# czbiohub-sf/shrimPy

Measured on AMD Instinct MI355X. Metric: voxels/sec deskew+20-iter RL deconv, 2048×2048×512 f32; HBM GB/s vs peak, higher is better.
Workload: dtype f32

## Files before the change

shrimpy_amd/csrc/rfft_rows.hip:

```cpp

#include "correlate_common.hpp"
#include "fft_lds.hpp"

namespace {

using namespace lsr_fft;

constexpr int kThreads = 512;
constexpr int kRows = 8;
constexpr int kPerRow = kThreads / kRows;
constexpr int kMaxM = 2048;
constexpr int kMaxTapsX = 2 * kPerRow + 1;

struct RowsArgs {
  const float* in;
  int Zi, Yi, Xi;
  float2* spec;
  int Z, Y, X, M, XC;
  const float2* tw_half;
  const float2* tw_x;
  Factors f;
  float* pval;
  unsigned long long* pidx;
  const float* aux;
  float* out;
  int Zo, Yo, Xo;
  float scale, eps;
  int pz, py, px;
  const double* norm_table;
  float norm_full;
  double* stats;
};

__device__ __forceinline__ int reflect_index(int i, int n) {
  if (n == 1) return 0;
  const int period = 2 * (n - 1);
  i = i % period;
  if (i < 0) i += period;
  return i < n ? i : period - i;
}
__device__ __forceinline__ int match_index(int o, int ni, int no) {
  if (no > ni) return reflect_index(o - (no - ni) / 2, ni);
  return o + (ni - no) / 2;
}

struct Tile {
  float2* buf;
  float2* tw;
  int pitch;
};

__device__ __forceinline__ Tile carve(float2* smem, int M) {
  Tile t;
  t.pitch = M + 1;
  t.buf = smem;
  t.tw = smem + kRows * t.pitch;
  return t;
}

__device__ __forceinline__ float2 tw_m(const float2* tw, int half, int i) {
  const bool hi = i >= half;
  const float2 v = tw[hi ? i - half : i];
  return hi ? float2{-v.x, -v.y} : v;
}

__device__ __forceinline__ int xcd_tile(int n_tiles, int block) {
  const int per = (n_tiles + 7) >> 3;
  const int t = (block & 7) * per + (block >> 3);
  return t < n_tiles ? t : -1;
}
__host__ __device__ inline unsigned xcd_grid(int64_t n_tiles) { return static_cast<unsigned>(8 * ((n_tiles + 7) / 8)); }

__device__ __forceinline__ void store_zero_tile(const RowsArgs& p, int z, int y0, int nrows, int tid) {
  const int r = tid & (kRows - 1), k0 = tid / kRows;
  if (r < nrows) {
    float2* out = p.spec + static_cast<int64_t>(z) * p.XC * p.Y + y0 + r;
    for (int k = k0; k <= p.M; k += kThreads / kRows) out[static_cast<int64_t>(k) * p.Y] = float2{0.0f, 0.0f};
  }
}

__device__ __forceinline__ void r2c_post_store(const RowsArgs& p, const Tile& t, int z, int y0, int nrows, int tid) {
  const int M = p.M;
  const int r = tid & (kRows - 1), k0 = tid / kRows;
  if (r < nrows) {
    const float2* row = t.buf + r * t.pitch;
    float2* out = p.spec + static_cast<int64_t>(z) * p.XC * p.Y + y0 + r;
    const float2* twx = p.tw_x;
    const int64_t ystride = p.Y;
    batched_loop<8>(k0, M + 1, kThreads / kRows, [twx](int k) { return twx[k]; },
                    [row, out, M, ystride](int k, float2 w) {
                      const float2 a = row[k == M ? 0 : k], b = cconj(row[k == 0 ? 0 : M - k]);
                      const float2 e = float2{0.5f * (a.x + b.x), 0.5f * (a.y + b.y)};
                      const float2 o = mul_mi(float2{0.5f * (a.x - b.x), 0.5f * (a.y - b.y)});
                      out[static_cast<int64_t>(k) * ystride] = cadd(e, cmul(w, o));
                    });
  }
}

template <bool ZERO>
__global__ __launch_bounds__(kThreads) void rfft_rows_kernel(RowsArgs p) {
  extern __shared__ float2 smem[];
  const int M = p.M, half = M / 2;
  const Tile t = carve(smem, M);
  const int tid = threadIdx.x;
  const int tiles_y = (p.Y + kRows - 1) / kRows;
  int z, y0;
  if constexpr (ZERO) {
    const int ty_src = (p.Yi + kRows - 1) / kRows, n_src = p.Zi * ty_src;
    const int first_pad = static_cast<int>(xcd_grid(n_src));
    if (static_cast<int>(blockIdx.x) < first_pad) {
      const int tile = xcd_tile(n_src, blockIdx.x);
      if (tile < 0) return;
      z = tile / ty_src;
      y0 = (tile - z * ty_src) * kRows;
    } else {
      const int q = static_cast<int>(blockIdx.x) - first_pad, beside = tiles_y - ty_src, n_beside = p.Zi * beside;
      if (q >= n_beside) return;
      z = q / beside;
      y0 = (ty_src + q - z * beside) * kRows;
    }
  } else {
    const int tile = xcd_tile(p.Z * tiles_y, blockIdx.x);
    if (tile < 0) return;
    z = tile / tiles_y;
    y0 = (tile - z * tiles_y) * kRows;
  }
  const int nrows = min(kRows, p.Y - y0);

  if constexpr (ZERO) {
    if (z >= p.Zi || y0 >= p.Yi) {
      store_zero_tile(p, z, y0, nrows, tid);
      return;
    }
  }
  for (int k = tid; k < half; k += kThreads) t.tw[k] = p.tw_half[k];
  if constexpr (ZERO) {
    const int r = tid / kPerRow, lane = tid & (kPerRow - 1);
    float2* row = t.buf + r * t.pitch;
    if (r < nrows && y0 + r < p.Yi) {
      const float* src = p.in + (static_cast<int64_t>(z) * p.Yi + y0 + r) * p.Xi;
      const int last = p.Xi - 1, n_src = (p.Xi + 1) / 2;
      batched_loop<8>(lane, n_src, kPerRow,
                      [src, last](int m) { return float2{src[2 * m], src[min(2 * m + 1, last)]}; },
                      [row, last](int m, float2 v) { row[m] = float2{v.x, 2 * m + 1 <= last ? v.y : 0.0f}; });
      for (int m = lane + ((n_src - lane + kPerRow - 1) / kPerRow) * kPerRow; m < M; m += kPerRow) row[m] = float2{0.0f, 0.0f};
    } else {
      for (int m = lane; m < M; m += kPerRow) row[m] = float2{0.0f, 0.0f};
    }
  } else {
    const int r = tid / kPerRow, lane = tid & (kPerRow - 1);
    float2* row = t.buf + r * t.pitch;
    if (r < nrows) {
      const float* src = p.in + (static_cast<int64_t>(match_index(z, p.Zi, p.Z)) * p.Yi + match_index(y0 + r, p.Yi, p.Y)) * p.Xi;
      const int shift = p.X > p.Xi ? -((p.X - p.Xi) / 2) : (p.Xi - p.X) / 2;
      const int xi = p.Xi;
      batched_loop<8>(lane, M, kPerRow,
                      [src, shift, xi](int m) {
                        const int x0 = 2 * m + shift, x1 = x0 + 1;
                        const bool inside = x0 >= 0 && x1 < xi;
                        return float2{src[inside ? x0 : reflect_index(x0, xi)], src[inside ? x1 : reflect_index(x1, xi)]};
                      },
                      [row](int m, float2 v) { row[m] = v; });
    } else {
      for (int m = lane; m < M; m += kPerRow) row[m] = float2{0.0f, 0.0f};
    }
  }
  __syncthreads();

  const float2* twl = t.tw;
  transform<kMaxM, kPerRow>(t.buf + (tid / kPerRow) * t.pitch, M, p.f, [twl, half](int i) { return tw_m(twl, half, i); },
                            tid & (kPerRow - 1));

  __syncthreads();
  r2c_post_store(p, t, z, y0, nrows, tid);
}

__device__ __forceinline__ void load_spectrum_tile(const RowsArgs& p, const Tile& t, int z, int y0, int y_end, int tid) {
  const int M = p.M;
  const int r = tid & (kRows - 1), k0 = tid / kRows;
  float2* row = t.buf + r * t.pitch;
  if (y0 + r < y_end) {
    const float2* in = p.spec + static_cast<int64_t>(z) * p.XC * p.Y + y0 + r;
    const int64_t ystride = p.Y;
    batched_loop<10>(k0, M + 1, kThreads / kRows, [in, ystride](int k) { return in[static_cast<int64_t>(k) * ystride]; },
                     [row](int k, float2 v) { row[k] = v; });
  } else {
    for (int k = k0; k <= M; k += kThreads / kRows) row[k] = float2{0.0f, 0.0f};
  }
}

__device__ __forceinline__ void c2r_pre_step(const RowsArgs& p, const Tile& t, int tid) {
  const int M = p.M, half = M / 2;
  const int r = tid / kPerRow, lane = tid & (kPerRow - 1);
  float2* row = t.buf + r * t.pitch;
  const float2* twx = p.tw_x;
  struct Pair { float2 a, b; };
  batched_loop<5>(lane, half + 1, kPerRow, [twx, M](int m) { return Pair{twx[m], twx[M - m]}; },
                  [row, M](int m, Pair w) {
                    const int mm = M - m;
                    const float2 xa = row[m], xb = row[mm];
                    const float2 wa = cconj(w.a), wb = cconj(w.b);
                    const float2 za = cadd(cadd(xa, cconj(xb)), mul_i(cmul(wa, csub(xa, cconj(xb)))));
                    const float2 zb = cadd(cadd(xb, cconj(xa)), mul_i(cmul(wb, csub(xb, cconj(xa)))));
                    row[m] = cconj(za);
                    if (m != 0 && mm != m) row[mm] = cconj(zb);
                  });
}

__device__ __forceinline__ void peak_merge(float& v, unsigned long long& i, float v2, unsigned long long i2) {
  if (v2 > v || (v2 == v && i2 < i)) { v = v2; i = i2; }
}

__global__ __launch_bounds__(kThreads) void irfft_rows_peak_kernel(RowsArgs p) {
  extern __shared__ float2 smem[];
  const int M = p.M, half = M / 2;
  const Tile t = carve(smem, M);
  unsigned long long* const s_i = reinterpret_cast<unsigned long long*>(smem);
  float* const s_v = reinterpret_cast<float*>(smem + kThreads);
  const int tid = threadIdx.x;
  const int tiles_y = (p.Y + kRows - 1) / kRows;
  const int z = blockIdx.x / tiles_y, y0 = (blockIdx.x - z * tiles_y) * kRows;
  const int nrows = min(kRows, p.Y - y0);

  for (int k = tid; k < half; k += kThreads) t.tw[k] = p.tw_half[k];
  load_spectrum_tile(p, t, z, y0, p.Y, tid);
  __syncthreads();
  c2r_pre_step(p, t, tid);
  __syncthreads();

  const float2* twl = t.tw;
  transform<kMaxM, kPerRow>(t.buf + (tid / kPerRow) * t.pitch, M, p.f, [twl, half](int i) { return tw_m(twl, half, i); },
                            tid & (kPerRow - 1));

  float best = -1.0f;
  unsigned long long best_i = ~0ull;
  {
    const int r = tid / kPerRow, lane = tid & (kPerRow - 1);
    if (r < nrows) {
      const float2* row = t.buf + r * t.pitch;
      const int y = y0 + r;
      const int zs = (z + p.Z / 2) % p.Z, ys = (y + p.Y / 2) % p.Y;
      const unsigned long long base = (static_cast<unsigned long long>(zs) * p.Y + ys) * p.X;
      for (int m = lane; m < M; m += kPerRow) {
        const float2 v = row[m];
        const float a = fabsf(v.x), b = fabsf(v.y);
        if (a >= best) peak_merge(best, best_i, a, base + static_cast<unsigned>((2 * m + p.X / 2) % p.X));
        if (b >= best) peak_merge(best, best_i, b, base + static_cast<unsigned>((2 * m + 1 + p.X / 2) % p.X));
      }
    }
  }
  __syncthreads();
  s_v[tid] = best;
  s_i[tid] = best_i;
  __syncthreads();
  for (int w = kThreads / 2; w > 0; w >>= 1) {
    if (tid < w) peak_merge(s_v[tid], s_i[tid], s_v[tid + w], s_i[tid + w]);
    __syncthreads();
  }
  if (tid == 0) {
    p.pval[blockIdx.x] = s_v[0];
    p.pidx[blockIdx.x] = s_i[0];
  }
}

__device__ __forceinline__ float rl_border_norm(const RowsArgs& p, int z, int y, int x) {
  const double* P = p.norm_table;
  const int cz = p.pz / 2, cy = p.py / 2, cx = p.px / 2;
  const int a0 = max(0, cz - z), a1 = min(p.pz, p.Zo - z + cz);
  const int b0 = max(0, cy - y), b1 = min(p.py, p.Yo - y + cy);
  const int c0 = max(0, cx - x), c1 = min(p.px, p.Xo - x + cx);
  const int sb = p.px + 1, sa = (p.py + 1) * sb;
  return static_cast<float>(((P[a1 * sa + b1 * sb + c1] - P[a0 * sa + b1 * sb + c1]) -
                             (P[a1 * sa + b0 * sb + c1] - P[a0 * sa + b0 * sb + c1])) -
                            ((P[a1 * sa + b1 * sb + c0] - P[a0 * sa + b1 * sb + c0]) -
                             (P[a1 * sa + b0 * sb + c0] - P[a0 * sa + b0 * sb + c0])));
}

template <int EPI, bool STATS, bool CHAIN = false>
__global__ __launch_bounds__(kThreads) void irfft_rows_rl_kernel(RowsArgs p) {
  extern __shared__ float2 smem[];
  const int M = p.M, half = M / 2;
  const Tile t = carve(smem, M);
  const int tid = threadIdx.x;
  const int ty_out = (p.Yo + kRows - 1) / kRows, n_out = p.Zo * ty_out;
  int z, y0;
  if (!CHAIN || static_cast<int>(blockIdx.x) < static_cast<int>(xcd_grid(n_out))) {
    const int tile = xcd_tile(n_out, blockIdx.x);
    if (tile < 0) return;
    z = tile / ty_out;
    y0 = (tile - z * ty_out) * kRows;
  } else {
    const int tiles_y = (p.Y + kRows - 1) / kRows;
    const int q = static_cast<int>(blockIdx.x) - static_cast<int>(xcd_grid(n_out)), beside = tiles_y - ty_out;
    const int n_beside = p.Zo * beside;
    if (q < n_beside) {
      z = q / beside;
      y0 = (ty_out + q - z * beside) * kRows;
      store_zero_tile(p, z, y0, min(kRows, p.Y - y0), tid);
    }
    return;
  }
  const int nrows = min(kRows, p.Yo - y0);

  for (int k = tid; k < half; k += kThreads) t.tw[k] = p.tw_half[k];
  load_spectrum_tile(p, t, z, y0, p.Y, tid);
  __syncthreads();
  c2r_pre_step(p, t, tid);
  __syncthreads();

  float n_left[2] = {1.0f, 1.0f}, n_right[2] = {1.0f, 1.0f}, n_row = 1.0f;
  int m_right = -1;
  if constexpr (EPI == LSR_EPI_UPDATE) {
    const int r = tid / kPerRow, lane = tid & (kPerRow - 1);
    if (r < nrows) {
      const int y = y0 + r;
      const int cz = p.pz / 2, cy = p.py / 2, cx = p.px / 2;
      const bool zy_inside = z >= cz && z < p.Zo - cz && y >= cy && y < p.Yo - cy;
      n_row = zy_inside ? p.norm_full : rl_border_norm(p, z, y, min(cx, p.Xo - 1));
      const int m_lo = max(p.Xo - cx, 0) >> 1, m_hi = (p.Xo - 1) >> 1;
      m_right = m_lo + ((lane - m_lo) & (kPerRow - 1));
      if (m_right > m_hi) m_right = -1;
#pragma unroll
      for (int h = 0; h < 2; ++h) {
        const int xl = 2 * lane + h, xr = 2 * m_right + h;
        n_left[h] = (xl < cx && xl < p.Xo) ? rl_border_norm(p, z, y, xl) : n_row;
        n_right[h] = (m_right >= 0 && xr >= p.Xo - cx && xr < p.Xo) ? rl_border_norm(p, z, y, xr) : n_row;
      }
    }
  }

  const float2* twl = t.tw;
  transform<kMaxM, kPerRow>(t.buf + (tid / kPerRow) * t.pitch, M, p.f, [twl, half](int i) { return tw_m(twl, half, i); },
                            tid & (kPerRow - 1));

  lsr::RlStats stats;
  {
    const int r = tid / kPerRow, lane = tid & (kPerRow - 1);
    if (r < nrows) {
      float2* row = t.buf + r * t.pitch;
      const int y = y0 + r;
      const int64_t base = (static_cast<int64_t>(z) * p.Yo + y) * p.Xo;
      const float* aux = p.aux + base;
      float* out = p.out == nullptr ? nullptr : p.out + base;
      const int cx = p.px / 2;
      const int last = p.Xo - 1;
      batched_loop<6>(lane, (p.Xo + 1) / 2, kPerRow,
                      [aux, last](int m) { return float2{aux[2 * m], aux[min(2 * m + 1, last)]}; },
                      [&](int m, float2 av) {
        const float2 c = row[m];
        const float v[2] = {c.x * p.scale, -c.y * p.scale};
        const float a2[2] = {av.x, av.y};
        float res[2] = {0.0f, 0.0f};
#pragma unroll
        for (int h = 0; h < 2; ++h) {
          const int x = 2 * m + h;
          if (x < p.Xo) {
            const float a = a2[h];
            if constexpr (EPI == LSR_EPI_RATIO) {
              res[h] = a / (fmaxf(v[h], 0.0f) + p.eps);
              if (!CHAIN || out != nullptr) out[x] = res[h];
            } else {
              const float nrm = (m == lane && x < cx) ? n_left[h] : ((m == m_right && x >= p.Xo - cx) ? n_right[h] : n_row);
              const float xu = a * v[h];
              res[h] = xu / nrm;
              out[x] = res[h];
              if constexpr (STATS) stats.add(a, xu, res[h]);
            }
          }
        }
        if constexpr (CHAIN) row[m] = float2{res[0], res[1]};
      });
      if constexpr (CHAIN) {
        const int n_src = (p.Xo + 1) / 2;
        for (int m = lane + ((n_src - lane + kPerRow - 1) / kPerRow) * kPerRow; m < M; m += kPerRow) row[m] = float2{0.0f, 0.0f};
      }
    } else if constexpr (CHAIN) {
      float2* row = t.buf + r * t.pitch;
      for (int m = lane; m < M; m += kPerRow) row[m] = float2{0.0f, 0.0f};
    }
  }
  if constexpr (CHAIN) {
    __syncthreads();
    transform<kMaxM, kPerRow>(t.buf + (tid / kPerRow) * t.pitch, M, p.f, [twl, half](int i) { return tw_m(twl, half, i); },
                              tid & (kPerRow - 1));
    __syncthreads();
    r2c_post_store(p, t, z, y0, min(kRows, p.Y - y0), tid);
  }
  if constexpr (STATS) lsr::rl_stats_flush<kThreads / 64>(stats, reinterpret_cast<float*>(smem), p.stats);
}

__global__ __launch_bounds__(256) void rows_peak_final_kernel(const float* __restrict__ pval,
                                                             const unsigned long long* __restrict__ pidx, int64_t nb,
                                                             long long* __restrict__ out) {
  __shared__ float s_v[256];
  __shared__ unsigned long long s_i[256];
  float best = -1.0f;
  unsigned long long best_i = ~0ull;
  for (int64_t i = threadIdx.x; i < nb; i += 256) peak_merge(best, best_i, pval[i], pidx[i]);
  s_v[threadIdx.x] = best;
  s_i[threadIdx.x] = best_i;
  __syncthreads();
  for (int w = 128; w > 0; w >>= 1) {
    if (static_cast<int>(threadIdx.x) < w) peak_merge(s_v[threadIdx.x], s_i[threadIdx.x], s_v[threadIdx.x + w], s_i[threadIdx.x + w]);
    __syncthreads();
  }
  if (threadIdx.x == 0) out[0] = static_cast<long long>(s_i[0]);
}

int fill(RowsArgs& p, int64_t Z, int64_t Y, int64_t X, const float* tw_half, const float* tw_x) {
  LSR_REQUIRE(Z > 0 && Y > 0 && X > 0, LSR_E_SHAPE, "grid (%lld,%lld,%lld) must be positive", (long long)Z, (long long)Y,
              (long long)X);
  LSR_REQUIRE_VOLUME(Z, Y, X);
  LSR_REQUIRE(lsr_rfft_rows_supported(X), LSR_E_UNSUPPORTED,
              "row length %lld: a multiple of 4 whose half is 5-smooth and at most %d", (long long)X, kMaxM);
  LSR_REQUIRE_PTR(tw_half);
  LSR_REQUIRE_PTR(tw_x);
  const int64_t lim = int64_t(1) << 30;
  LSR_REQUIRE(Z < lim && Y < lim, LSR_E_UNSUPPORTED, "a dimension exceeds 2^30");
  p.Z = static_cast<int>(Z); p.Y = static_cast<int>(Y); p.X = static_cast<int>(X);
  p.M = p.X / 2; p.XC = p.M + 1;
  p.tw_half = reinterpret_cast<const float2*>(tw_half);
  p.tw_x = reinterpret_cast<const float2*>(tw_x);
  LSR_REQUIRE(factorize(p.M, &p.f), LSR_E_UNSUPPORTED, "row length %lld has too many factors", (long long)X);
  LSR_REQUIRE(Z * lsr::ceil_div(Y, kRows) < (int64_t(1) << 31), LSR_E_SHAPE, "grid of workgroups is too large");
  return LSR_OK;
}

size_t lds_bytes(int M) {
  const size_t tile = (static_cast<size_t>(kRows) * (M + 1) + M / 2) * sizeof(float2);
  const size_t reduction = static_cast<size_t>(kThreads) * (sizeof(unsigned long long) + sizeof(float));
  return tile > reduction ? tile : reduction;
}

template <typename K>
int allow_lds(K kernel, std::atomic<uint64_t>& done, const char* what) {
  return lsr::allow_dynamic_lds(reinterpret_cast<const void*>(kernel), static_cast<int>(lds_bytes(kMaxM)), done, what);
}

}

extern "C" int lsr_rfft_rows_supported(int64_t n) {
  if (n < 8 || n % 4 != 0 || n / 2 > kMaxM) return 0;
  int64_t m = n / 2;
  for (int f : {2, 3, 5})
    while (m % f == 0) m /= f;
  return m == 1 && lsr::lds_fits(lds_bytes(static_cast<int>(n / 2)));
}

extern "C" int64_t lsr_rfft_rows_scratch_bytes(int64_t Z, int64_t Y) {
  if (!lsr::volume_in_range(Z, Y, 1)) return -1;
  return Z * lsr::ceil_div(Y, kRows) * 16;
}

extern "C" int lsr_rfft_rows_t_c64(const float* in, int64_t Zi, int64_t Yi, int64_t Xi, float* spec, int64_t Z, int64_t Y,
                                   int64_t X, const float* tw_half, const float* tw_x, lsr_stream_t stream) {
  LSR_REQUIRE_PTR(in);
  LSR_REQUIRE_PTR(spec);
  LSR_REQUIRE(Zi > 0 && Yi > 0 && Xi > 0, LSR_E_SHAPE, "source shape (%lld,%lld,%lld) must be positive", (long long)Zi,
              (long long)Yi, (long long)Xi);
  LSR_REQUIRE_VOLUME(Zi, Yi, Xi);
  const int64_t lim = int64_t(1) << 30;
  LSR_REQUIRE(Zi < lim && Yi < lim && Xi < lim, LSR_E_UNSUPPORTED, "a dimension exceeds 2^30");
  LSR_REQUIRE((Z <= Zi || Z - Zi < 2 * Zi - 1) && (Y <= Yi || Y - Yi < 2 * Yi - 1) && (X <= Xi || X - Xi < 2 * Xi - 1),
              LSR_E_ARG, "reflect padding from (%lld,%lld,%lld) to (%lld,%lld,%lld) exceeds the source size", (long long)Zi,
              (long long)Yi, (long long)Xi, (long long)Z, (long long)Y, (long long)X);
  RowsArgs p{};
  if (int rc = fill(p, Z, Y, X, tw_half, tw_x)) return rc;
  p.in = in;
  p.Zi = static_cast<int>(Zi); p.Yi = static_cast<int>(Yi); p.Xi = static_cast<int>(Xi);
  p.spec = reinterpret_cast<float2*>(spec);
  static std::atomic<uint64_t> lds_allowed{0};
  if (int rc = allow_lds(rfft_rows_kernel<false>, lds_allowed, "lsr_rfft_rows_t_c64")) return rc;
  const unsigned blocks = xcd_grid(Z * lsr::ceil_div(Y, kRows));
  hipLaunchKernelGGL(rfft_rows_kernel<false>, dim3(blocks), dim3(kThreads), lds_bytes(p.M), lsr::as_stream(stream), p);
  return lsr::launch_status("lsr_rfft_rows_t_c64");
}

extern "C" int lsr_irfft_rows_peak(const float* spec, int64_t Z, int64_t Y, int64_t X, const float* tw_half,
                                   const float* tw_x, long long* out_index, void* scratch, lsr_stream_t stream) {
  LSR_REQUIRE_PTR(spec);
  LSR_REQUIRE_PTR(out_index);
  LSR_REQUIRE_PTR(scratch);
  RowsArgs p{};
  if (int rc = fill(p, Z, Y, X, tw_half, tw_x)) return rc;
  p.spec = const_cast<float2*>(reinterpret_cast<const float2*>(spec));
  const int64_t nb = Z * lsr::ceil_div(Y, kRows);
  p.pidx = static_cast<unsigned long long*>(scratch);
  p.pval = reinterpret_cast<float*>(static_cast<char*>(scratch) + 8 * nb);
  static std::atomic<uint64_t> lds_allowed{0};
  if (int rc = allow_lds(irfft_rows_peak_kernel, lds_allowed, "lsr_irfft_rows_peak")) return rc;
  hipStream_t s = lsr::as_stream(stream);
  hipLaunchKernelGGL(irfft_rows_peak_kernel, dim3(static_cast<unsigned>(nb)), dim3(kThreads), lds_bytes(p.M), s, p);
  hipLaunchKernelGGL(rows_peak_final_kernel, dim3(1), dim3(256), 0, s, p.pval, p.pidx, nb, out_index);
  return lsr::launch_status("lsr_irfft_rows_peak");
}

extern "C" int lsr_rfft_rows_zero_t_c64(const float* in, int64_t Zi, int64_t Yi, int64_t Xi, float* spec, int64_t Z,
                                        int64_t Y, int64_t X, const float* tw_half, const float* tw_x,
                                        lsr_stream_t stream) {
  LSR_REQUIRE_PTR(in);
  LSR_REQUIRE_PTR(spec);
  LSR_REQUIRE(Zi > 0 && Yi > 0 && Xi > 0, LSR_E_SHAPE, "source shape (%lld,%lld,%lld) must be positive", (long long)Zi,
              (long long)Yi, (long long)Xi);
  LSR_REQUIRE_VOLUME(Zi, Yi, Xi);
  LSR_REQUIRE(Zi <= Z && Yi <= Y && Xi <= X, LSR_E_SHAPE, "the source (%lld,%lld,%lld) must fit the grid (%lld,%lld,%lld)",
              (long long)Zi, (long long)Yi, (long long)Xi, (long long)Z, (long long)Y, (long long)X);
  RowsArgs p{};
  if (int rc = fill(p, Z, Y, X, tw_half, tw_x)) return rc;
  p.in = in;
  p.Zi = static_cast<int>(Zi); p.Yi = static_cast<int>(Yi); p.Xi = static_cast<int>(Xi);
  p.spec = reinterpret_cast<float2*>(spec);
  static std::atomic<uint64_t> lds_allowed{0};
  if (int rc = allow_lds(rfft_rows_kernel<true>, lds_allowed, "lsr_rfft_rows_zero_t_c64")) return rc;
  const int64_t src_tiles = Zi * lsr::ceil_div(Yi, kRows), beside = Zi * (lsr::ceil_div(Y, kRows) - lsr::ceil_div(Yi, kRows));
  const unsigned blocks = xcd_grid(src_tiles) + static_cast<unsigned>(beside);
  hipLaunchKernelGGL(rfft_rows_kernel<true>, dim3(blocks), dim3(kThreads), lds_bytes(p.M), lsr::as_stream(stream), p);
  return lsr::launch_status("lsr_rfft_rows_zero_t_c64");
}

extern "C" int lsr_irfft_rows_rl_f32(const float* spec, int64_t Z, int64_t Y, int64_t X, const float* tw_half,
                                     const float* tw_x, int epilogue, const float* aux, float* out, int64_t Zo, int64_t Yo,
                                     int64_t Xo, float scale, float eps, int pz, int py, int px, const double* norm_table,
                                     float norm_full, double* stats, lsr_stream_t stream) {
  LSR_REQUIRE_PTR(spec);
  LSR_REQUIRE_PTR(aux);
  LSR_REQUIRE_PTR(out);
  LSR_REQUIRE(epilogue == LSR_EPI_RATIO || epilogue == LSR_EPI_UPDATE, LSR_E_ARG,
              "epilogue must be LSR_EPI_RATIO or LSR_EPI_UPDATE, got %d", epilogue);
  LSR_REQUIRE(Zo > 0 && Yo > 0 && Xo > 0 && Zo <= Z && Yo <= Y && Xo <= X, LSR_E_SHAPE,
              "the volume (%lld,%lld,%lld) must be positive and fit the grid (%lld,%lld,%lld)", (long long)Zo, (long long)Yo,
              (long long)Xo, (long long)Z, (long long)Y, (long long)X);
  LSR_REQUIRE(scale > 0.0f && eps > 0.0f, LSR_E_ARG, "scale and eps must be positive");
  RowsArgs p{};
  if (int rc = fill(p, Z, Y, X, tw_half, tw_x)) return rc;
  if (epilogue == LSR_EPI_UPDATE) {
    LSR_REQUIRE_PTR(norm_table);
    LSR_REQUIRE(pz > 0 && py > 0 && px > 0 && pz % 2 == 1 && py % 2 == 1 && px % 2 == 1 && pz < 4096 && py < 4096 &&
                    px < 4096, LSR_E_ARG, "PSF extents (%d,%d,%d) must be odd and positive", pz, py, px);
    LSR_REQUIRE(norm_full > 0.0f, LSR_E_ARG, "norm_full must be positive");
    LSR_REQUIRE(px <= kMaxTapsX, LSR_E_UNSUPPORTED, "PSF of %d taps along x: the border normalisation covers at most %d",
                px, kMaxTapsX);
  }
  p.spec = const_cast<float2*>(reinterpret_cast<const float2*>(spec));
  p.aux = aux; p.out = out;
  p.Zo = static_cast<int>(Zo); p.Yo = static_cast<int>(Yo); p.Xo = static_cast<int>(Xo);
  p.scale = scale; p.eps = eps;
  p.pz = pz; p.py = py; p.px = px;
  p.norm_table = norm_table; p.norm_full = norm_full; p.stats = stats;
  const unsigned blocks = xcd_grid(Zo * lsr::ceil_div(Yo, kRows));
  hipStream_t s = lsr::as_stream(stream);
  static std::atomic<uint64_t> a0{0}, a1{0}, a2{0};
  if (epilogue == LSR_EPI_RATIO) {
    if (int rc = allow_lds(irfft_rows_rl_kernel<LSR_EPI_RATIO, false>, a0, "lsr_irfft_rows_rl_f32")) return rc;
    hipLaunchKernelGGL((irfft_rows_rl_kernel<LSR_EPI_RATIO, false>), dim3(blocks), dim3(kThreads), lds_bytes(p.M), s, p);
  } else if (stats == nullptr) {
    if (int rc = allow_lds(irfft_rows_rl_kernel<LSR_EPI_UPDATE, false>, a1, "lsr_irfft_rows_rl_f32")) return rc;
    hipLaunchKernelGGL((irfft_rows_rl_kernel<LSR_EPI_UPDATE, false>), dim3(blocks), dim3(kThreads), lds_bytes(p.M), s, p);
  } else {
    if (int rc = allow_lds(irfft_rows_rl_kernel<LSR_EPI_UPDATE, true>, a2, "lsr_irfft_rows_rl_f32")) return rc;
    hipLaunchKernelGGL((irfft_rows_rl_kernel<LSR_EPI_UPDATE, true>), dim3(blocks), dim3(kThreads), lds_bytes(p.M), s, p);
  }
  return lsr::launch_status("lsr_irfft_rows_rl_f32");
}

extern "C" int lsr_rl_rows_chain_f32(float* spec, int64_t Z, int64_t Y, int64_t X, const float* tw_half, const float* tw_x,
                                     int epilogue, const float* aux, float* out, int64_t Zo, int64_t Yo, int64_t Xo,
                                     float scale, float eps, int pz, int py, int px, const double* norm_table,
                                     float norm_full, double* stats, lsr_stream_t stream) {
  LSR_REQUIRE_PTR(spec);
  LSR_REQUIRE_PTR(aux);
  LSR_REQUIRE(epilogue == LSR_EPI_RATIO || epilogue == LSR_EPI_UPDATE, LSR_E_ARG,
              "epilogue must be LSR_EPI_RATIO or LSR_EPI_UPDATE, got %d", epilogue);
  if (epilogue == LSR_EPI_UPDATE) LSR_REQUIRE_PTR(out);
  LSR_REQUIRE(Zo > 0 && Yo > 0 && Xo > 0 && Zo <= Z && Yo <= Y && Xo <= X, LSR_E_SHAPE,
              "the volume (%lld,%lld,%lld) must be positive and fit the grid (%lld,%lld,%lld)", (long long)Zo, (long long)Yo,
              (long long)Xo, (long long)Z, (long long)Y, (long long)X);
  LSR_REQUIRE(scale > 0.0f && eps > 0.0f, LSR_E_ARG, "scale and eps must be positive");
  RowsArgs p{};
  if (int rc = fill(p, Z, Y, X, tw_half, tw_x)) return rc;
  if (epilogue == LSR_EPI_UPDATE) {
    LSR_REQUIRE_PTR(norm_table);
    LSR_REQUIRE(pz > 0 && py > 0 && px > 0 && pz % 2 == 1 && py % 2 == 1 && px % 2 == 1 && pz < 4096 && py < 4096 &&
                    px < 4096, LSR_E_ARG, "PSF extents (%d,%d,%d) must be odd and positive", pz, py, px);
    LSR_REQUIRE(norm_full > 0.0f, LSR_E_ARG, "norm_full must be positive");
    LSR_REQUIRE(px <= kMaxTapsX, LSR_E_UNSUPPORTED, "PSF of %d taps along x: the border normalisation covers at most %d",
                px, kMaxTapsX);
  }
  p.spec = reinterpret_cast<float2*>(spec);
  p.aux = aux; p.out = out;
  p.Zo = static_cast<int>(Zo); p.Yo = static_cast<int>(Yo); p.Xo = static_cast<int>(Xo);
  p.scale = scale; p.eps = eps;
  p.pz = pz; p.py = py; p.px = px;
  p.norm_table = norm_table; p.norm_full = norm_full; p.stats = stats;
  const int64_t out_tiles = Zo * lsr::ceil_div(Yo, kRows), beside = Zo * (lsr::ceil_div(Y, kRows) - lsr::ceil_div(Yo, kRows));
  const unsigned blocks = xcd_grid(out_tiles) + static_cast<unsigned>(beside);
  hipStream_t s = lsr::as_stream(stream);
  static std::atomic<uint64_t> a0{0}, a1{0}, a2{0};
  if (epilogue == LSR_EPI_RATIO) {
    if (int rc = allow_lds(irfft_rows_rl_kernel<LSR_EPI_RATIO, false, true>, a0, "lsr_rl_rows_chain_f32")) return rc;
    hipLaunchKernelGGL((irfft_rows_rl_kernel<LSR_EPI_RATIO, false, true>), dim3(blocks), dim3(kThreads), lds_bytes(p.M), s, p);
  } else if (stats == nullptr) {
    if (int rc = allow_lds(irfft_rows_rl_kernel<LSR_EPI_UPDATE, false, true>, a1, "lsr_rl_rows_chain_f32")) return rc;
    hipLaunchKernelGGL((irfft_rows_rl_kernel<LSR_EPI_UPDATE, false, true>), dim3(blocks), dim3(kThreads), lds_bytes(p.M), s, p);
  } else {
    if (int rc = allow_lds(irfft_rows_rl_kernel<LSR_EPI_UPDATE, true, true>, a2, "lsr_rl_rows_chain_f32")) return rc;
    hipLaunchKernelGGL((irfft_rows_rl_kernel<LSR_EPI_UPDATE, true, true>), dim3(blocks), dim3(kThreads), lds_bytes(p.M), s, p);
  }
  return lsr::launch_status("lsr_rl_rows_chain_f32");
}
```

shrimpy_amd/csrc/zcorr.hip:

```cpp

#include "fft_lds.hpp"

#include <cstdlib>

namespace {

using namespace lsr_fft;

constexpr int kThreads = 256;
constexpr int kCols = 16;
constexpr int kPerCol = kThreads / kCols;
constexpr int kMaxN = 256;

struct ZcorrArgs {
  const float2* f1;
  float2* g;
  const float2* tw;
  int N, Y, XC;
  Factors f;
  float inv_n;
  int mode;
  int z_valid, z_keep;
};

__global__ __launch_bounds__(kThreads) void zcorr_kernel(ZcorrArgs p) {
  extern __shared__ float2 smem[];
  const int N = p.N, pitch = N + 1;
  float2* buf = smem;
  float2* tw = smem + kCols * pitch;
  const int tid = threadIdx.x;
  const int tiles_y = (p.Y + kCols - 1) / kCols;
  const int xc = blockIdx.x / tiles_y, y0 = (blockIdx.x - xc * tiles_y) * kCols;
  const int ncols = min(kCols, p.Y - y0);

  for (int k = tid; k < N; k += kThreads) tw[k] = p.tw[k];
  const int c = tid & (kCols - 1), z0 = tid / kCols;
  const int64_t row = static_cast<int64_t>(p.XC) * p.Y;
  const float2* g = p.g + static_cast<int64_t>(xc) * p.Y + y0 + c;
  if (c < ncols) {
    float2* col = buf + c * pitch;
    batched_loop<8>(z0, p.z_valid, kThreads / kCols, [g, row](int z) { return g[z * row]; }, [col](int z, float2 v) { col[z] = v; });
    for (int z = z0 + ((p.z_valid - z0 + kThreads / kCols - 1) / (kThreads / kCols)) * (kThreads / kCols); z < N; z += kThreads / kCols)
      col[z] = float2{0.0f, 0.0f};
  } else {
    for (int z = z0; z < N; z += kThreads / kCols) buf[c * pitch + z] = float2{0.0f, 0.0f};
  }
  __syncthreads();

  float2* const my_col = buf + (tid / kPerCol) * pitch;
  const int t = tid & (kPerCol - 1);
  const float2* f1 = p.f1 + (static_cast<int64_t>(xc) * p.Y + y0) * N;
  const int my = tid / kPerCol;
  for (int round = 0; round < 2; ++round) {
    transform<kMaxN, kPerCol>(my_col, N, p.f, [tw](int i) { return tw[i]; }, t);
    if (round == 0) {
      if (my < ncols) {
        const float2* ref = f1 + static_cast<int64_t>(my) * N;
        const int mode = p.mode;
        batched_loop<8>(t, N, kPerCol, [ref](int k) { return ref[k]; }, [my_col, mode](int k, float2 f) {
          if (mode == 0) my_col[k] = cmul(cconj(f), my_col[k]);
          else if (mode == 1) my_col[k] = cconj(cmul(f, my_col[k]));
          else my_col[k] = cmul(f, cconj(my_col[k]));
        });
      }
      sequence_sync();
    }
  }
  __syncthreads();

  float2* out = p.g + static_cast<int64_t>(xc) * p.Y + y0 + c;
  if (c < ncols)
    for (int z = z0; z < p.z_keep; z += kThreads / kCols) out[z * row] = cconj(buf[c * pitch + z]);
}

}

extern "C" int lsr_cross_correlate_z_supported(int64_t n) {
  if (n < 2 || n > kMaxN) return 0;
  const size_t lds = (static_cast<size_t>(kCols) * (n + 1) + n) * sizeof(float2);
  for (int f : {2, 3, 5})
    while (n % f == 0) n /= f;
  return n == 1 && lsr::lds_fits(lds);
}

namespace {
int z_leg(const float* f1, float* g, const float* twiddles, int64_t N, int64_t Y, int64_t XC, int mode, int64_t z_valid,
          int64_t z_keep, lsr_stream_t stream);
}

extern "C" int lsr_cross_correlate_z_c64(const float* f1, float* g, const float* twiddles, int64_t N, int64_t Y, int64_t XC,
                                         lsr_stream_t stream) {
  return z_leg(f1, g, twiddles, N, Y, XC, 0, N, N, stream);
}

extern "C" int lsr_spectrum_multiply_z_c64(const float* f1, float* g, const float* twiddles, int64_t N, int64_t Y,
                                           int64_t XC, int conj_f1, int64_t z_valid, int64_t z_keep, lsr_stream_t stream) {
  LSR_REQUIRE(conj_f1 == 0 || conj_f1 == 1, LSR_E_ARG, "conj_f1 must be 0 or 1, got %d", conj_f1);
  LSR_REQUIRE(z_valid >= 1 && z_valid <= N && z_keep >= 1 && z_keep <= N, LSR_E_ARG,
              "z_valid %lld and z_keep %lld must lie in [1, N = %lld]", (long long)z_valid, (long long)z_keep, (long long)N);
  return z_leg(f1, g, twiddles, N, Y, XC, conj_f1 ? 2 : 1, z_valid, z_keep, stream);
}

namespace {
int z_leg(const float* f1, float* g, const float* twiddles, int64_t N, int64_t Y, int64_t XC, int mode, int64_t z_valid,
          int64_t z_keep, lsr_stream_t stream) {
  LSR_REQUIRE_PTR(f1);
  LSR_REQUIRE_PTR(g);
  LSR_REQUIRE_PTR(twiddles);
  LSR_REQUIRE(N > 0 && Y > 0 && XC > 0, LSR_E_SHAPE, "shape (%lld,%lld,%lld) must be positive", (long long)N, (long long)Y,
              (long long)XC);
  LSR_REQUIRE_VOLUME(N, Y, XC);
  LSR_REQUIRE(lsr_cross_correlate_z_supported(N), LSR_E_UNSUPPORTED,
              "z length %lld: this kernel transforms 5-smooth lengths from 2 to %d", (long long)N, kMaxN);
  LSR_REQUIRE((reinterpret_cast<uintptr_t>(f1) & 7) == 0 && (reinterpret_cast<uintptr_t>(g) & 7) == 0 &&
                  (reinterpret_cast<uintptr_t>(twiddles) & 7) == 0, LSR_E_ARG, "complex64 arrays must be 8-byte aligned");
  ZcorrArgs p;
  p.f1 = reinterpret_cast<const float2*>(f1);
  p.g = reinterpret_cast<float2*>(g);
  p.tw = reinterpret_cast<const float2*>(twiddles);
  p.N = static_cast<int>(N); p.Y = static_cast<int>(Y); p.XC = static_cast<int>(XC);
  LSR_REQUIRE(factorize(N, &p.f), LSR_E_UNSUPPORTED, "z length %lld has more than %d factors", (long long)N, kMaxFactors);
  if (const char* e = std::getenv("LSR_ZCORR_ORDER")) {
    int f[kMaxFactors], k = 0;
    long long prod = 1;
    for (const char* c = e; *c && k < kMaxFactors;) {
      const int v = std::atoi(c);
      if (v != 2 && v != 3 && v != 4 && v != 5) { k = 0; break; }
      f[k++] = v;
      prod *= v;
      while (*c && *c != ',') ++c;
      if (*c == ',') ++c;
    }
    if (k > 0 && prod == N) {
      p.f.n = k;
      for (int i = 0, stride = 1; i < k; ++i) {
        p.f.radix[i] = f[i];
        p.f.inv_stride[i] = 1.0f / static_cast<float>(stride);
        stride *= f[i];
      }
    }
  }
  p.inv_n = 1.0f / static_cast<float>(p.N);
  p.mode = mode;
  p.z_valid = static_cast<int>(z_valid); p.z_keep = static_cast<int>(z_keep);
  const int64_t blocks = XC * lsr::ceil_div(Y, kCols);
  LSR_REQUIRE(blocks < (int64_t(1) << 31), LSR_E_SHAPE, "grid of %lld workgroups is too large", (long long)blocks);
  const size_t lds = (static_cast<size_t>(kCols) * (p.N + 1) + p.N) * sizeof(float2);
  static std::atomic<uint64_t> lds_allowed{0};
  if (int rc = lsr::allow_dynamic_lds(reinterpret_cast<const void*>(zcorr_kernel),
                                      static_cast<int>((kCols * (kMaxN + 1) + kMaxN) * sizeof(float2)), lds_allowed,
                                      "lsr_cross_correlate_z_c64"))
    return rc;
  hipLaunchKernelGGL(zcorr_kernel, dim3(static_cast<unsigned>(blocks)), dim3(kThreads), lds, lsr::as_stream(stream), p);
  return lsr::launch_status("lsr_cross_correlate_z_c64");
}
}
```

Measured before the change: 40.76 billion.

## Prefetch row tiles into registers before twiddle staging for short FFT lengths

Adds a register-held prefetch path, compiled when the row FFT length is at most 1152, in the zero-padded forward rfft and the inverse RL row kernels. All global loads for a tile are issued up front into registers, then the twiddle table is staged into LDS, and only then are the held values written to LDS, so load latency overlaps the twiddle copy. Kernels are now templated on the maximum FFT length so the short variant can size its register arrays and unrolls; the host picks the variant from M. The z-correlation loads are also deepened from 8 to 12 in flight. The cost is higher register pressure and possible occupancy loss, plus more kernel instantiations.

```diff
diff --git a/shrimpy_amd/csrc/rfft_rows.hip b/shrimpy_amd/csrc/rfft_rows.hip
--- a/shrimpy_amd/csrc/rfft_rows.hip
+++ b/shrimpy_amd/csrc/rfft_rows.hip
@@ -11,6 +11,7 @@
 constexpr int kPerRow = kThreads / kRows;
 constexpr int kMaxM = 2048;
 constexpr int kMaxTapsX = 2 * kPerRow + 1;
+constexpr int kShortM = 1152;
 
 struct RowsArgs {
   const float* in;
@@ -70,7 +71,6 @@
   return t < n_tiles ? t : -1;
 }
 __host__ __device__ inline unsigned xcd_grid(int64_t n_tiles) { return static_cast<unsigned>(8 * ((n_tiles + 7) / 8)); }
-
 __device__ __forceinline__ void store_zero_tile(const RowsArgs& p, int z, int y0, int nrows, int tid) {
   const int r = tid & (kRows - 1), k0 = tid / kRows;
   if (r < nrows) {
@@ -97,57 +97,19 @@
   }
 }
 
-template <bool ZERO>
 __global__ __launch_bounds__(kThreads) void rfft_rows_kernel(RowsArgs p) {
   extern __shared__ float2 smem[];
   const int M = p.M, half = M / 2;
   const Tile t = carve(smem, M);
   const int tid = threadIdx.x;
   const int tiles_y = (p.Y + kRows - 1) / kRows;
-  int z, y0;
-  if constexpr (ZERO) {
-    const int ty_src = (p.Yi + kRows - 1) / kRows, n_src = p.Zi * ty_src;
-    const int first_pad = static_cast<int>(xcd_grid(n_src));
-    if (static_cast<int>(blockIdx.x) < first_pad) {
-      const int tile = xcd_tile(n_src, blockIdx.x);
-      if (tile < 0) return;
-      z = tile / ty_src;
-      y0 = (tile - z * ty_src) * kRows;
-    } else {
-      const int q = static_cast<int>(blockIdx.x) - first_pad, beside = tiles_y - ty_src, n_beside = p.Zi * beside;
-      if (q >= n_beside) return;
-      z = q / beside;
-      y0 = (ty_src + q - z * beside) * kRows;
-    }
-  } else {
-    const int tile = xcd_tile(p.Z * tiles_y, blockIdx.x);
-    if (tile < 0) return;
-    z = tile / tiles_y;
-    y0 = (tile - z * tiles_y) * kRows;
-  }
+  const int tile = xcd_tile(p.Z * tiles_y, blockIdx.x);
+  if (tile < 0) return;
+  const int z = tile / tiles_y, y0 = (tile - z * tiles_y) * kRows;
   const int nrows = min(kRows, p.Y - y0);
 
-  if constexpr (ZERO) {
-    if (z >= p.Zi || y0 >= p.Yi) {
-      store_zero_tile(p, z, y0, nrows, tid);
-      return;
-    }
-  }
   for (int k = tid; k < half; k += kThreads) t.tw[k] = p.tw_half[k];
-  if constexpr (ZERO) {
-    const int r = tid / kPerRow, lane = tid & (kPerRow - 1);
-    float2* row = t.buf + r * t.pitch;
-    if (r < nrows && y0 + r < p.Yi) {
-      const float* src = p.in + (static_cast<int64_t>(z) * p.Yi + y0 + r) * p.Xi;
-      const int last = p.Xi - 1, n_src = (p.Xi + 1) / 2;
-      batched_loop<8>(lane, n_src, kPerRow,
-                      [src, last](int m) { return float2{src[2 * m], src[min(2 * m + 1, last)]}; },
-                      [row, last](int m, float2 v) { row[m] = float2{v.x, 2 * m + 1 <= last ? v.y : 0.0f}; });
-      for (int m = lane + ((n_src - lane + kPerRow - 1) / kPerRow) * kPerRow; m < M; m += kPerRow) row[m] = float2{0.0f, 0.0f};
-    } else {
-      for (int m = lane; m < M; m += kPerRow) row[m] = float2{0.0f, 0.0f};
-    }
-  } else {
+  {
     const int r = tid / kPerRow, lane = tid & (kPerRow - 1);
     float2* row = t.buf + r * t.pitch;
     if (r < nrows) {
@@ -175,6 +137,86 @@
   r2c_post_store(p, t, z, y0, nrows, tid);
 }
 
+template <int SLOTS, bool HELD>
+struct Held {
+  float2 v[HELD ? SLOTS : 1];
+};
+
+template <int SLOTS, bool HELD>
+__device__ __forceinline__ void request_source_tile(const RowsArgs& p, Held<SLOTS, HELD>& h, int z, int y0, int tid) {
+  if constexpr (HELD) {
+    const int r = tid / kPerRow, lane = tid & (kPerRow - 1);
+    const float* src = p.in + (static_cast<int64_t>(z) * p.Yi + min(y0 + r, p.Yi - 1)) * p.Xi;
+    const int last = p.Xi - 1, n_src = (p.Xi + 1) / 2;
+#pragma unroll
+    for (int k = 0; k < SLOTS; ++k) {
+      const int m = min(lane + k * kPerRow, n_src - 1);
+      h.v[k] = float2{src[2 * m], src[min(2 * m + 1, last)]};
+    }
+  }
+}
+
+template <int SLOTS, bool HELD>
+__device__ __forceinline__ void place_source_tile(const RowsArgs& p, const Tile& t, const Held<SLOTS, HELD>& h, int z, int y0,
+                                                  int tid) {
+  const int M = p.M;
+  const int r = tid / kPerRow, lane = tid & (kPerRow - 1);
+  float2* row = t.buf + r * t.pitch;
+  const int last = p.Xi - 1, n_src = (p.Xi + 1) / 2;
+  if constexpr (HELD) {
+    const bool live = y0 + r < p.Yi;
+#pragma unroll
+    for (int k = 0; k < SLOTS; ++k) {
+      const int m = lane + k * kPerRow;
+      const float2 v = h.v[k];
+      if (m < M) row[m] = float2{live && m < n_src ? v.x : 0.0f, live && 2 * m + 1 <= last ? v.y : 0.0f};
+    }
+  } else if (y0 + r < p.Yi) {
+    const float* src = p.in + (static_cast<int64_t>(z) * p.Yi + y0 + r) * p.Xi;
+    batched_loop<8>(lane, n_src, kPerRow,
+                    [src, last](int m) { return float2{src[2 * m], src[min(2 * m + 1, last)]}; },
+                    [row, last](int m, float2 v) { row[m] = float2{v.x, 2 * m + 1 <= last ? v.y : 0.0f}; });
+    for (int m = lane + ((n_src - lane + kPerRow - 1) / kPerRow) * kPerRow; m < M; m += kPerRow) row[m] = float2{0.0f, 0.0f};
+  } else {
+    for (int m = lane; m < M; m += kPerRow) row[m] = float2{0.0f, 0.0f};
+  }
+}
+
+template <int MAXM>
+__global__ __launch_bounds__(kThreads) void rfft_rows_zero_kernel(RowsArgs p) {
+  extern __shared__ float2 smem[];
+  constexpr bool HELD = MAXM <= kShortM;
+  const int M = p.M, half = M / 2;
+  const Tile t = carve(smem, M);
+  const int tid = threadIdx.x;
+  const int tiles_y = (p.Y + kRows - 1) / kRows;
+  const int ty_src = (p.Yi + kRows - 1) / kRows, n_src = p.Zi * ty_src;
+  const int first_pad = static_cast<int>(xcd_grid(n_src));
+  if (static_cast<int>(blockIdx.x) >= first_pad) {
+    const int q = static_cast<int>(blockIdx.x) - first_pad, beside = tiles_y - ty_src;
+    if (q >= p.Zi * beside) return;
+    const int z = q / beside, y0 = (ty_src + q - z * beside) * kRows;
+    store_zero_tile(p, z, y0, min(kRows, p.Y - y0), tid);
+    return;
+  }
+  const int tile = xcd_tile(n_src, blockIdx.x);
+  if (tile < 0) return;
+  const int z = tile / ty_src, y0 = (tile - z * ty_src) * kRows;
+
+  Held<MAXM / kPerRow, HELD> held;
+  request_source_tile(p, held, z, y0, tid);
+  for (int k = tid; k < half; k += kThreads) t.tw[k] = p.tw_half[k];
+  place_source_tile(p, t, held, z, y0, tid);
+  __syncthreads();
+
+  const float2* twl = t.tw;
+  transform<MAXM, kPerRow>(t.buf + (tid / kPerRow) * t.pitch, M, p.f, [twl, half](int i) { return tw_m(twl, half, i); },
+                           tid & (kPerRow - 1));
+
+  __syncthreads();
+  r2c_post_store(p, t, z, y0, min(kRows, p.Y - y0), tid);
+}
+
 __device__ __forceinline__ void load_spectrum_tile(const RowsArgs& p, const Tile& t, int z, int y0, int y_end, int tid) {
   const int M = p.M;
   const int r = tid & (kRows - 1), k0 = tid / kRows;
@@ -186,6 +228,34 @@
                      [row](int k, float2 v) { row[k] = v; });
   } else {
     for (int k = k0; k <= M; k += kThreads / kRows) row[k] = float2{0.0f, 0.0f};
+  }
+}
+
+template <int SLOTS, bool HELD>
+__device__ __forceinline__ void request_spectrum_tile(const RowsArgs& p, Held<SLOTS, HELD>& h, int z, int y0, int tid) {
+  if constexpr (HELD) {
+    const int r = tid & (kRows - 1), k0 = tid / kRows;
+    const float2* in = p.spec + static_cast<int64_t>(z) * p.XC * p.Y + min(y0 + r, p.Y - 1);
+    const int64_t ystride = p.Y;
+#pragma unroll
+    for (int j = 0; j < SLOTS; ++j) h.v[j] = in[static_cast<int64_t>(min(k0 + j * (kThreads / kRows), p.M)) * ystride];
+  }
+}
+template <int SLOTS, bool HELD>
+__device__ __forceinline__ void place_spectrum_tile(const RowsArgs& p, const Tile& t, const Held<SLOTS, HELD>& h, int z, int y0,
+                                                    int tid) {
+  if constexpr (HELD) {
+    const int r = tid & (kRows - 1), k0 = tid / kRows;
+    float2* row = t.buf + r * t.pitch;
+    const bool live = y0 + r < p.Y;
+#pragma unroll
+    for (int j = 0; j < SLOTS; ++j) {
+      const int k = k0 + j * (kThreads / kRows);
+      const float2 v = h.v[j];
+      if (k <= p.M) row[k] = float2{live ? v.x : 0.0f, live ? v.y : 0.0f};
+    }
+  } else {
+    load_spectrum_tile(p, t, z, y0, p.Y, tid);
   }
 }
 
@@ -276,9 +346,10 @@
                              (P[a1 * sa + b0 * sb + c0] - P[a0 * sa + b0 * sb + c0])));
 }
 
-template <int EPI, bool STATS, bool CHAIN = false>
+template <int EPI, bool STATS, bool CHAIN, int MAXM>
 __global__ __launch_bounds__(kThreads) void irfft_rows_rl_kernel(RowsArgs p) {
   extern __shared__ float2 smem[];
+  constexpr bool HELD = MAXM <= kShortM;
   const int M = p.M, half = M / 2;
   const Tile t = carve(smem, M);
   const int tid = threadIdx.x;
@@ -302,8 +373,10 @@
   }
   const int nrows = min(kRows, p.Yo - y0);
 
+  Held<MAXM / (kThreads / kRows) + 1, HELD> held;
+  request_spectrum_tile(p, held, z, y0, tid);
   for (int k = tid; k < half; k += kThreads) t.tw[k] = p.tw_half[k];
-  load_spectrum_tile(p, t, z, y0, p.Y, tid);
+  place_spectrum_tile(p, t, held, z, y0, tid);
   __syncthreads();
   c2r_pre_step(p, t, tid);
   __syncthreads();
@@ -330,8 +403,8 @@
   }
 
   const float2* twl = t.tw;
-  transform<kMaxM, kPerRow>(t.buf + (tid / kPerRow) * t.pitch, M, p.f, [twl, half](int i) { return tw_m(twl, half, i); },
-                            tid & (kPerRow - 1));
+  transform<MAXM, kPerRow>(t.buf + (tid / kPerRow) * t.pitch, M, p.f, [twl, half](int i) { return tw_m(twl, half, i); },
+                           tid & (kPerRow - 1));
 
   lsr::RlStats stats;
   {
@@ -344,7 +417,7 @@
       float* out = p.out == nullptr ? nullptr : p.out + base;
       const int cx = p.px / 2;
       const int last = p.Xo - 1;
-      batched_loop<6>(lane, (p.Xo + 1) / 2, kPerRow,
+      batched_loop<HELD ? MAXM / kPerRow : 6>(lane, (p.Xo + 1) / 2, kPerRow,
                       [aux, last](int m) { return float2{aux[2 * m], aux[min(2 * m + 1, last)]}; },
                       [&](int m, float2 av) {
         const float2 c = row[m];
@@ -381,8 +454,8 @@
   }
   if constexpr (CHAIN) {
     __syncthreads();
-    transform<kMaxM, kPerRow>(t.buf + (tid / kPerRow) * t.pitch, M, p.f, [twl, half](int i) { return tw_m(twl, half, i); },
-                              tid & (kPerRow - 1));
+    transform<MAXM, kPerRow>(t.buf + (tid / kPerRow) * t.pitch, M, p.f, [twl, half](int i) { return tw_m(twl, half, i); },
+                             tid & (kPerRow - 1));
     __syncthreads();
     r2c_post_store(p, t, z, y0, min(kRows, p.Y - y0), tid);
   }
@@ -435,6 +508,25 @@
 template <typename K>
 int allow_lds(K kernel, std::atomic<uint64_t>& done, const char* what) {
   return lsr::allow_dynamic_lds(reinterpret_cast<const void*>(kernel), static_cast<int>(lds_bytes(kMaxM)), done, what);
+}
+
+template <int EPI, bool STATS, bool CHAIN>
+int launch_rl_as(const RowsArgs& p, unsigned blocks, hipStream_t s, const char* what) {
+  static std::atomic<uint64_t> a0{0}, a1{0};
+  if (p.M <= kShortM) {
+    if (int rc = allow_lds(irfft_rows_rl_kernel<EPI, STATS, CHAIN, kShortM>, a0, what)) return rc;
+    hipLaunchKernelGGL((irfft_rows_rl_kernel<EPI, STATS, CHAIN, kShortM>), dim3(blocks), dim3(kThreads), lds_bytes(p.M), s, p);
+  } else {
+    if (int rc = allow_lds(irfft_rows_rl_kernel<EPI, STATS, CHAIN, kMaxM>, a1, what)) return rc;
+    hipLaunchKernelGGL((irfft_rows_rl_kernel<EPI, STATS, CHAIN, kMaxM>), dim3(blocks), dim3(kThreads), lds_bytes(p.M), s, p);
+  }
+  return lsr::launch_status(what);
+}
+template <bool CHAIN>
+int launch_rl(const RowsArgs& p, unsigned blocks, int epilogue, hipStream_t s, const char* what) {
+  if (epilogue == LSR_EPI_RATIO) return launch_rl_as<LSR_EPI_RATIO, false, CHAIN>(p, blocks, s, what);
+  if (p.stats == nullptr) return launch_rl_as<LSR_EPI_UPDATE, false, CHAIN>(p, blocks, s, what);
+  return launch_rl_as<LSR_EPI_UPDATE, true, CHAIN>(p, blocks, s, what);
 }
 
 }
@@ -470,9 +562,9 @@
   p.Zi = static_cast<int>(Zi); p.Yi = static_cast<int>(Yi); p.Xi = static_cast<int>(Xi);
   p.spec = reinterpret_cast<float2*>(spec);
   static std::atomic<uint64_t> lds_allowed{0};
-  if (int rc = allow_lds(rfft_rows_kernel<false>, lds_allowed, "lsr_rfft_rows_t_c64")) return rc;
+  if (int rc = allow_lds(rfft_rows_kernel, lds_allowed, "lsr_rfft_rows_t_c64")) return rc;
   const unsigned blocks = xcd_grid(Z * lsr::ceil_div(Y, kRows));
-  hipLaunchKernelGGL(rfft_rows_kernel<false>, dim3(blocks), dim3(kThreads), lds_bytes(p.M), lsr::as_stream(stream), p);
+  hipLaunchKernelGGL(rfft_rows_kernel, dim3(blocks), dim3(kThreads), lds_bytes(p.M), lsr::as_stream(stream), p);
   return lsr::launch_status("lsr_rfft_rows_t_c64");
 }
 
@@ -510,11 +602,16 @@
   p.in = in;
   p.Zi = static_cast<int>(Zi); p.Yi = static_cast<int>(Yi); p.Xi = static_cast<int>(Xi);
   p.spec = reinterpret_cast<float2*>(spec);
-  static std::atomic<uint64_t> lds_allowed{0};
-  if (int rc = allow_lds(rfft_rows_kernel<true>, lds_allowed, "lsr_rfft_rows_zero_t_c64")) return rc;
   const int64_t src_tiles = Zi * lsr::ceil_div(Yi, kRows), beside = Zi * (lsr::ceil_div(Y, kRows) - lsr::ceil_div(Yi, kRows));
   const unsigned blocks = xcd_grid(src_tiles) + static_cast<unsigned>(beside);
-  hipLaunchKernelGGL(rfft_rows_kernel<true>, dim3(blocks), dim3(kThreads), lds_bytes(p.M), lsr::as_stream(stream), p);
+  static std::atomic<uint64_t> a0{0}, a1{0};
+  if (p.M <= kShortM) {
+    if (int rc = allow_lds(rfft_rows_zero_kernel<kShortM>, a0, "lsr_rfft_rows_zero_t_c64")) return rc;
+    hipLaunchKernelGGL(rfft_rows_zero_kernel<kShortM>, dim3(blocks), dim3(kThreads), lds_bytes(p.M), lsr::as_stream(stream), p);
+  } else {
+    if (int rc = allow_lds(rfft_rows_zero_kernel<kMaxM>, a1, "lsr_rfft_rows_zero_t_c64")) return rc;
+    hipLaunchKernelGGL(rfft_rows_zero_kernel<kMaxM>, dim3(blocks), dim3(kThreads), lds_bytes(p.M), lsr::as_stream(stream), p);
+  }
   return lsr::launch_status("lsr_rfft_rows_zero_t_c64");
 }
 
@@ -547,20 +644,7 @@
   p.scale = scale; p.eps = eps;
   p.pz = pz; p.py = py; p.px = px;
   p.norm_table = norm_table; p.norm_full = norm_full; p.stats = stats;
-  const unsigned blocks = xcd_grid(Zo * lsr::ceil_div(Yo, kRows));
-  hipStream_t s = lsr::as_stream(stream);
-  static std::atomic<uint64_t> a0{0}, a1{0}, a2{0};
-  if (epilogue == LSR_EPI_RATIO) {
-    if (int rc = allow_lds(irfft_rows_rl_kernel<LSR_EPI_RATIO, false>, a0, "lsr_irfft_rows_rl_f32")) return rc;
-    hipLaunchKernelGGL((irfft_rows_rl_kernel<LSR_EPI_RATIO, false>), dim3(blocks), dim3(kThreads), lds_bytes(p.M), s, p);
-  } else if (stats == nullptr) {
-    if (int rc = allow_lds(irfft_rows_rl_kernel<LSR_EPI_UPDATE, false>, a1, "lsr_irfft_rows_rl_f32")) return rc;
-    hipLaunchKernelGGL((irfft_rows_rl_kernel<LSR_EPI_UPDATE, false>), dim3(blocks), dim3(kThreads), lds_bytes(p.M), s, p);
-  } else {
-    if (int rc = allow_lds(irfft_rows_rl_kernel<LSR_EPI_UPDATE, true>, a2, "lsr_irfft_rows_rl_f32")) return rc;
-    hipLaunchKernelGGL((irfft_rows_rl_kernel<LSR_EPI_UPDATE, true>), dim3(blocks), dim3(kThreads), lds_bytes(p.M), s, p);
-  }
-  return lsr::launch_status("lsr_irfft_rows_rl_f32");
+  return launch_rl<false>(p, xcd_grid(Zo * lsr::ceil_div(Yo, kRows)), epilogue, lsr::as_stream(stream), "lsr_irfft_rows_rl_f32");
 }
 
 extern "C" int lsr_rl_rows_chain_f32(float* spec, int64_t Z, int64_t Y, int64_t X, const float* tw_half, const float* tw_x,
@@ -593,18 +677,6 @@
   p.pz = pz; p.py = py; p.px = px;
   p.norm_table = norm_table; p.norm_full = norm_full; p.stats = stats;
   const int64_t out_tiles = Zo * lsr::ceil_div(Yo, kRows), beside = Zo * (lsr::ceil_div(Y, kRows) - lsr::ceil_div(Yo, kRows));
-  const unsigned blocks = xcd_grid(out_tiles) + static_cast<unsigned>(beside);
-  hipStream_t s = lsr::as_stream(stream);
-  static std::atomic<uint64_t> a0{0}, a1{0}, a2{0};
-  if (epilogue == LSR_EPI_RATIO) {
-    if (int rc = allow_lds(irfft_rows_rl_kernel<LSR_EPI_RATIO, false, true>, a0, "lsr_rl_rows_chain_f32")) return rc;
-    hipLaunchKernelGGL((irfft_rows_rl_kernel<LSR_EPI_RATIO, false, true>), dim3(blocks), dim3(kThreads), lds_bytes(p.M), s, p);
-  } else if (stats == nullptr) {
-    if (int rc = allow_lds(irfft_rows_rl_kernel<LSR_EPI_UPDATE, false, true>, a1, "lsr_rl_rows_chain_f32")) return rc;
-    hipLaunchKernelGGL((irfft_rows_rl_kernel<LSR_EPI_UPDATE, false, true>), dim3(blocks), dim3(kThreads), lds_bytes(p.M), s, p);
-  } else {
-    if (int rc = allow_lds(irfft_rows_rl_kernel<LSR_EPI_UPDATE, true, true>, a2, "lsr_rl_rows_chain_f32")) return rc;
-    hipLaunchKernelGGL((irfft_rows_rl_kernel<LSR_EPI_UPDATE, true, true>), dim3(blocks), dim3(kThreads), lds_bytes(p.M), s, p);
-  }
-  return lsr::launch_status("lsr_rl_rows_chain_f32");
-}
+  return launch_rl<true>(p, xcd_grid(out_tiles) + static_cast<unsigned>(beside), epilogue, lsr::as_stream(stream),
+                         "lsr_rl_rows_chain_f32");
+}
diff --git a/shrimpy_amd/csrc/zcorr.hip b/shrimpy_amd/csrc/zcorr.hip
--- a/shrimpy_amd/csrc/zcorr.hip
+++ b/shrimpy_amd/csrc/zcorr.hip
@@ -39,7 +39,7 @@
   const float2* g = p.g + static_cast<int64_t>(xc) * p.Y + y0 + c;
   if (c < ncols) {
     float2* col = buf + c * pitch;
-    batched_loop<8>(z0, p.z_valid, kThreads / kCols, [g, row](int z) { return g[z * row]; }, [col](int z, float2 v) { col[z] = v; });
+    batched_loop<12>(z0, p.z_valid, kThreads / kCols, [g, row](int z) { return g[z * row]; }, [col](int z, float2 v) { col[z] = v; });
     for (int z = z0 + ((p.z_valid - z0 + kThreads / kCols - 1) / (kThreads / kCols)) * (kThreads / kCols); z < N; z += kThreads / kCols)
       col[z] = float2{0.0f, 0.0f};
   } else {
@@ -57,7 +57,7 @@
       if (my < ncols) {
         const float2* ref = f1 + static_cast<int64_t>(my) * N;
         const int mode = p.mode;
-        batched_loop<8>(t, N, kPerCol, [ref](int k) { return ref[k]; }, [my_col, mode](int k, float2 f) {
+        batched_loop<12>(t, N, kPerCol, [ref](int k) { return ref[k]; }, [my_col, mode](int k, float2 f) {
           if (mode == 0) my_col[k] = cmul(cconj(f), my_col[k]);
           else if (mode == 1) my_col[k] = cconj(cmul(f, my_col[k]));
           else my_col[k] = cmul(f, cconj(my_col[k]));
```

Result: no change. 40.68 billion (-0.2%).
